# zhuwsh/ORB-SLAM2

Measured on AMD Instinct MI355X. Metric: frames/sec ORB extract+match, 1241x376 @1000 feats; bit-exact vs CPU, higher is better.
Workload: dtype u8; 1 GPU; KITTI-shape stereo 1241x376, nFeatures=1000/eye, 8 levels, FAST 20/7: extract(L)+extract(R)+ComputeStereoMatches; 1 frame = 1 stereo pair; images RESIDENT IN HBM when the timed region starts (kernel throughput: excludes PCIe; fed from pinned host memory the same path runs at config.host_fed_batched_frames_per_s -- the PCIe Gen5 x16 link, 0.96 MB per frame -- and one camera stream at config.host_fe; parallelism=1 independent camera-stream batches, one per GPU, ranks_seen=1, backend=none

## Files before the change

### include/orbx.h

```cpp
#ifndef ORBX_H
#define ORBX_H
#include <stddef.h>
#include <stdint.h>

#ifdef __cplusplus
extern "C" {
#endif

#define ORBX_OK 0
#define ORBX_E_INVALID (-1)
#define ORBX_E_CAPACITY (-2)
#define ORBX_E_TOO_SMALL (-3)
#define ORBX_E_NO_DEVICE (-4)
#define ORBX_E_HIP (-5)

typedef struct {
    float x, y, size, angle, response;
    int32_t octave, class_id;
} orbx_keypoint;

typedef struct orbx_extractor orbx_extractor;

const char *orbx_last_error(void);
int orbx_device_count(void);
// ... 231 lines not shown

int orbx_search_by_projection_keyframe(int device, const orbx_frame_feats *cur, const orbx_proj_points *pts,
                                       const float *scale_factors, int nlevels, float th, int orb_dist,
                                       int check_orientation, int32_t *match_cur, int *nmatches);
int orbx_search_by_projection_sim3(int device, const orbx_frame_feats *kf, const orbx_proj_points *pts,
                                   const float *scale_factors, int nlevels, float th, int32_t *match_kf, int *nmatches);
int orbx_window_best(int device, const orbx_frame_feats *kf, const orbx_proj_points *pts, const float *scale_factors,
                     const float *inv_sigma2, int nlevels, float th, int chi2, int max_dist, int32_t *best_idx,
                     int32_t *best_dist, int *nfound);
int orbx_search_by_sim3(int device, const orbx_frame_feats *kf1, const orbx_frame_feats *kf2, const orbx_proj_points *pts12,
                        const orbx_proj_points *pts21, const float *scale_factors1, const float *scale_factors2, int nlevels,
                        float th, int32_t *match12, int *nfound);

int orbx_search_for_initialization(int device, const orbx_frame_feats *f1, const orbx_frame_feats *f2,
                                   const float *prev_matched_xy, int window_size, float nnratio, int check_orientation,
                                   int32_t *matches12, int *nmatches);

int orbx_undistort_keypoints(int device, const float *xy, int n, float fx, float fy, float cx, float cy,
                             const float *dist_coef, int ndist, float *xy_out);


int orbx_distinctive_descriptors(int device, const uint8_t *desc, const int32_t *off, int npoints, int32_t *best_idx);


enum { ORBX_STAGE_RESIZE = 0, ORBX_STAGE_FAST = 1, ORBX_STAGE_TREE = 2, ORBX_STAGE_DESC = 3,
       ORBX_STAGE_STEREO = 4, ORBX_STAGE_STEREO_CUT = 5, ORBX_STAGE_COUNT = 6 };
int orbx_profile_enable(orbx_extractor *e, int enable);
int orbx_profile_stages(orbx_extractor *e, unsigned stage_mask);
int orbx_profile_read(orbx_extractor *e, float *ms, int *launches, int reset);

int orbx_debug_candidates(orbx_extractor *e, int image_index, int level, int32_t *x, int32_t *y, int32_t *resp, int cap, int *n);
int orbx_debug_level_counts(orbx_extractor *e, int image_index, int32_t *counts );
int orbx_debug_fast_form(const orbx_extractor *e);
int orbx_debug_set_bow_form(int form);
int orbx_debug_set_match_items(int in_memory);
int orbx_debug_match_timing(double *out4);

#ifdef __cplusplus
}
#endif
#endif
```

### orb-slam2_amd/csrc/orbx_extract.hip

```cpp
#include "orbx_device.h"
#include <atomic>
#include "orb_pattern.inc"

#include <math.h>
#include <stdio.h>
#include <stdlib.h>
#include <string.h>
#include <chrono>

__constant__ uint32_t c_pat4[256];
__constant__ uint4 c_omask[64];

#define RS_PX 4
#define RS_TW (64 * RS_PX)
#ifndef RS_TH_LOG2
#define RS_TH_LOG2 3
#endif
#define RS_TH (1 << RS_TH_LOG2)
#define RS_NT 64
#define RS_PITCH 320
#define RS_ROWS (RS_TH == 16 ? 22 : 12)

struct ResizeArgs {
    int d_w, d_pitch, s_w, s_pitch, s_level0;
// ... 49 lines not shown
    asm volatile("s_waitcnt vmcnt(0)" ::: "memory");
    __syncthreads();
    const int d_w = A.d_w, d_pitch = A.d_pitch;
    int hp[RS_PX], hc[RS_PX];
#pragma unroll
    for (int i = 0; i < RS_PX; i++) hp[i] = hc[i] = 0;
    uint8_t *dcol = dst + x4;
#define EMIT(Y, B0, B1, HA) do { \
        const unsigned w0_ = (unsigned)(B0) << 16, w1_ = (unsigned)(B1) << 16; \
        uint32_t out_ = 0; \
        _Pragma("unroll") for (int i = 0; i < RS_PX; i++) out_ |= ((__umulhi(w0_, (unsigned)(HA)[i]) + __umulhi(w1_, (unsigned)hc[i]) + 2u) >> 2) << (8 * i); \
        if (x4 < d_w) *reinterpret_cast<uint32_t *>(dcol + (long long)(Y) * d_pitch) = out_; } while (0)
#pragma unroll
    for (int k = 0; k < RS_ROWS; k++) {
        if (k < nrows) {
#pragma unroll
            for (int i = 0; i < RS_PX; i++) {
                hp[i] = hc[i];
                hc[i] = (src_t[k * RS_PITCH + o0[i]] * a0[i] + src_t[k * RS_PITCH + o1[i]] * a1[i]) >> 4;
            }
            const int e = __builtin_amdgcn_readfirstlane((int)qs[k].x);
            if (e >= 0) {
                const int y = e & 0xFFF;
                if (!(e & 0x1000)) {
                    const int b0 = __builtin_amdgcn_readfirstlane((int)qs[k].y), b1 = __builtin_amdgcn_readfirstlane((int)qs[k].z);
                    if (e & 0x2000) EMIT(y, b0, b1, hc);
                    else EMIT(y, b0, b1, hp);
                }
                if (e & 0x4000) EMIT(y + 1, 2048, 0, hc);
            }
        }
    }
#undef EMIT
}

__global__ __launch_bounds__(256) void k_resize_direct(const Geom *__restrict__ g, int l, PyrRef pr,
                                                       uint8_t *__restrict__ pyr_w, const int16_t *__restrict__ tabs)
{
    const LevelGeom &D = g->lv[l];
    const LevelGeom &S = g->lv[l - 1];
    const int b = blockIdx.z;
    const int x4 = (blockIdx.x * 64 + (threadIdx.x & 63)) * 4;
    const int y = blockIdx.y * 4 + (threadIdx.x >> 6);
    if (y >= D.h || x4 >= D.pitch) return;
    int spitch;
    const uint8_t *src = orbx_level_ptr(pr, S, l - 1, b, &spitch);
    uint8_t *dst = pyr_w + (long long)b * pr.pyr_stride + D.pyr_off;
    if (D.resize_lds == 2) {
        const uint8_t *r0 = src + (long long)(2 * y) * spitch, *r1 = r0 + spitch;
        uint32_t out = 0;
#pragma unroll
        for (int i = 0; i < 4; i++) {
            const int x = x4 + i;
            if (x < D.w) out |= (uint32_t)((r0[2 * x] + r0[2 * x + 1] + r1[2 * x] + r1[2 * x + 1] + 2) >> 2) << (8 * i);
        }
        *reinterpret_cast<uint32_t *>(dst + (long long)y * D.pitch + x4) = out;
        return;
    }
    const int16_t *tx = tabs + D.tab_x, *ty = tabs + D.tab_y;
    const int sy0 = ty[4 * y], b0 = ty[4 * y + 1], b1 = ty[4 * y + 2];
    const int sy1 = sy0 + 1 < S.h ? sy0 + 1 : S.h - 1;
    const uint8_t *r0 = src + (long long)sy0 * spitch, *r1 = src + (long long)sy1 * spitch;
    uint32_t out = 0;
#pragma unroll
    for (int i = 0; i < 4; i++) {
        const int x = x4 + i;
// ... 1765 lines not shown
            std::vector<int> ext(n + 1, 0);
            for (int t = 0; t < tiles; t++)
                for (int k = 0; k <= n; k++) {
                    const size_t i = (size_t)k * tiles + t;
                    int16_t *r = &tabs[off + ((size_t)t * (n + 1) + k) * rec];
                    if (hi[i] > 32767) return false;
                    r[0] = (int16_t)lo[i]; r[1] = (int16_t)hi[i]; r[2] = (int16_t)own[i];
                    int extent = hi[i] - lo[i];
                    if (!axis) {
                        int div;
                        if (k == 0) {
                            const int pitch_lim = lo[i] + (((dim(first - 1) - lo[i]) + 3) & ~3);
                            const int ndw = (std::min(lo[i] + ((hi[i] - lo[i] + 3) & ~3), pitch_lim) - lo[i]) / 4;
                            r[3] = (int16_t)ndw; div = ndw; extent = 4 * ndw;
                        } else { div = (extent + 3) >> 2; extent = (extent + 3) & ~3; }
                        const unsigned magic = (unsigned)((0x100000000ull + (unsigned)div - 1) / (unsigned)div);
                        r[4] = (int16_t)(magic & 0xFFFF); r[5] = (int16_t)(magic >> 16);
                    }
                    ext[k] = std::max(ext[k], extent);
                }
            if (!axis) P.tiles_x = tiles; else P.tiles_y = tiles;
            ext_axis[axis] = ext;
        }
        for (int k = 0; k < n; k++) lds[k & 1] = std::max(lds[k & 1], (size_t)ext_axis[0][k] * ext_axis[1][k]);
        P.lds_b = (int)align_up(lds[0], 16);
        P.lds_bytes = P.lds_b + (int)align_up(lds[1], 16);
        if (P.lds_bytes > PG_LDS_LIMIT) return false;
        first += n; gi++;
    }
    e->n_pyr_groups = gi;
    return true;
}

int orbx_prepare_geometry(orbx_extractor *e, int w, int h)
{
    if (e->geom.w == w && e->geom.h == h) return ORBX_OK;
    if (w > e->max_w || h > e->max_h || w > ORBX_MAX_DIM || h > ORBX_MAX_DIM) {
        orbx_set_error("image %dx%d exceeds the extractor's maximum %dx%d", w, h, e->max_w, e->max_h);
        return ORBX_E_INVALID;
    }
    Geom G;
    memset(&G, 0, sizeof G);
    G.nlevels = e->nlevels; G.w = w; G.h = h;
    size_t tab_units = 0;
    for (int l = 0; l < e->nlevels; l++) {
        LevelGeom &L = G.lv[l];
        L.w = orbx_cv_round((float)w * e->isf[l]);
        L.h = orbx_cv_round((float)h * e->isf[l]);
        const int min_b = ORBX_MIN_BORDER, max_bx = L.w - ORBX_EDGE + 3, max_by = L.h - ORBX_EDGE + 3;
        const float width = (float)(max_bx - min_b), height = (float)(max_by - min_b);
        if (max_bx - min_b < 30 || max_by - min_b < 30) {
            orbx_set_error("level %d (%dx%d) is smaller than one 30-px FAST cell", l, L.w, L.h);
            return ORBX_E_TOO_SMALL;
        }
        L.n_cols = (int)(width / 30.f);
        L.n_rows = (int)(height / 30.f);
        L.w_cell = (int)ceilf(width / L.n_cols);
        L.h_cell = (int)ceilf(height / L.n_rows);
        if (L.w_cell > 59 || L.h_cell > 59) { orbx_set_error("internal: cell larger than 59"); return ORBX_E_INVALID; }
        L.n_cells = L.n_cols * L.n_rows;
        L.cell_base = G.total_cells;
        G.total_cells += L.n_cells;
        L.cand_cap = ((L.w_cell + 1) / 2) * ((L.h_cell + 1) / 2);
        L.cand_off = G.cand_total;
        G.cand_total += (long long)L.n_cells * L.cand_cap;
        L.quota = e->quota[l];
// ... 78 lines not shown
        }
        for (int y0 = 0; y0 < L.h && ok; y0 += RS_TH) {
            const int yl = (y0 + RS_TH < L.h ? y0 + RS_TH : L.h) - 1;
            const int smax = ty[4 * yl] + 1 < S.h - 1 ? ty[4 * yl] + 1 : S.h - 1;
            if (smax - ty[4 * y0] + 1 > RS_ROWS) ok = false;
        }
        L.resize_lds = (S.w == 2 * L.w && S.h == 2 * L.h) ? 2 : (ok && emit_ok[l] && L.h < 4096) ? 1 : 0;
        if (L.resize_lds != 1) continue;
        for (int by = 0, y0 = 0; y0 < L.h; by++, y0 += RS_TH) {
            int16_t *r = &tabs[L.tab_ty + (size_t)by * RS_TY_REC];
            const int yl = (y0 + RS_TH < L.h ? y0 + RS_TH : L.h) - 1;
            const int sy_min = ty[4 * y0], sy_max = ty[4 * yl] + 1 < S.h - 1 ? ty[4 * yl] + 1 : S.h - 1, nrows = sy_max - sy_min + 1;
            r[0] = (int16_t)sy_min; r[1] = (int16_t)nrows; r[2] = r[3] = 0;
            for (int k = 0; k < RS_ROWS; k++) {
                int16_t *q = r + 4 + 4 * k;
                q[0] = -1; q[1] = q[2] = q[3] = 0;
                if (k >= nrows) continue;
                const int16_t *t = &emit[l][4 * (size_t)(sy_min + k)];
                if (t[0] < 0) continue;
                const int y = t[0] & 0xFFF, in1 = y >= y0 && y <= yl, in2 = (t[0] & 0x4000) && y + 1 >= y0 && y + 1 <= yl;
                if (!in1 && !in2) continue;
                q[0] = (int16_t)(y | (t[0] & 0x2000) | (in1 ? 0 : 0x1000) | (in2 ? 0x4000 : 0)); q[1] = t[1]; q[2] = t[2];
            }
        }
        for (int bx = 0, x0 = 0; x0 < L.w; bx++, x0 += RS_TW) {
            int16_t *r = &tabs[L.tab_tx + 4 * (size_t)bx];
            const int xl = (x0 + RS_TW < L.w ? x0 + RS_TW : L.w) - 1;
            const int sx_min = tx[4 * x0], sx_max = tx[4 * xl] + 1 < S.w - 1 ? tx[4 * xl] + 1 : S.w - 1, need = sx_max - sx_min + 1;
            const int nfull = std::min((need + 15) >> 4, (S.w - sx_min) >> 4), tail = std::max(need - 16 * nfull, 0);
            r[0] = (int16_t)sx_min; r[1] = (int16_t)nfull; r[2] = (int16_t)tail; r[3] = 0;
        }
    }
    if (!build_pyr_groups(e, G, tabs)) e->n_pyr_groups = 0;
    std::vector<CellRec> cells(G.total_cells);
    for (int l = 0; l < e->nlevels; l++) {
        const LevelGeom &L = G.lv[l];
        const int max_bx = L.w - ORBX_MIN_BORDER, max_by = L.h - ORBX_MIN_BORDER;
        for (int ci = 0; ci < L.n_cells; ci++) {
            CellRec &c = cells[L.cell_base + ci];
            const int row = ci / L.n_cols, col = ci % L.n_cols;
            const int ini_y = ORBX_MIN_BORDER + row * L.h_cell, ini_x = ORBX_MIN_BORDER + col * L.w_cell;
            const int max_y = ini_y + L.h_cell + 6 < max_by ? ini_y + L.h_cell + 6 : max_by;
            const int max_x = ini_x + L.w_cell + 6 < max_bx ? ini_x + L.w_cell + 6 : max_bx;
            c.level = (short)l;
            c.ini_x = (short)ini_x; c.ini_y = (short)ini_y; c.tw = (short)(max_x - ini_x); c.th = (short)(max_y - ini_y);
            c.skip = (ini_y >= max_by - 3 || ini_x >= max_bx - 6 || c.tw - 6 <= 0 || c.th - 6 <= 0) ? 1 : 0;
            c.pitch = L.pitch; c.cand_cap = L.cand_cap; c.pyr_off = L.pyr_off;
            { const int gpr = (c.tw - 6 + 3) >> 2; c.gpr_magic = gpr > 0 ? 0xFFFFFFFFu / (unsigned)gpr + 1u : 0u; }
            c.cand_slot = L.cand_off + (long long)ci * L.cand_cap;
        }
    }
    std::vector<PairRec> pairs;
    {
        bool ok = true;
        for (int l = 0; l < e->nlevels; l++) if (G.lv[l].w_cell > 32 || G.lv[l].h_cell > 56) ok = false;
        G.fast2_ok = ok ? 1 : 0;
        G.total_pairs = 0;
        if (ok) {
            for (int grp = 0; grp < 2; grp++) {
                int max_th = 0, max_dh = 0;
                G.fast2_first[grp] = (int)pairs.size();
                for (int l = 0; l < e->nlevels; l++) {
                    const LevelGeom &L = G.lv[l];
                    if ((L.h_cell <= 32 ? 0 : 1) != grp) continue;
                    max_th = std::max(max_th, L.h_cell + 6); max_dh = std::max(max_dh, L.h_cell);
                    for (int row = 0; row < L.n_rows; row++)
// ... 162 lines not shown
        max_w < 1 || max_h < 1 || ini_th < 1 || min_th < 1 || ini_th > 255 || min_th > ini_th) {
        orbx_set_error("orbx_extractor_create: invalid parameter");
        return ORBX_E_INVALID;
    }
    int ndev = 0;
    if (hipGetDeviceCount(&ndev) != hipSuccess || ndev < 1 || device < 0 || device >= ndev) {
        orbx_set_error("no usable HIP device (requested %d of %d); liborbx has no CPU fallback", device, ndev);
        return ORBX_E_NO_DEVICE;
    }
    ORBX_HIP(hipSetDevice(device));
    orbx_extractor *e = new orbx_extractor();
    e->prof_mask = ~0u;
    orbx_extractor_set_cv_profile(e, ORBX_CV_PROFILE_3_2);
    e->device = device; e->nfeatures = nfeatures; e->nlevels = nlevels; e->ini_th = ini_th; e->min_th = min_th;
    e->scale_factor = scale_factor; e->max_w = max_w; e->max_h = max_h; e->max_batch = max_batch;
    {
        const char *env = getenv("ORBX_PYR_GROUP_MAX_IMAGES");
        e->pyr_group_max_images = env && *env ? atoi(env) : 8;
        const char *mid = getenv("ORBX_PYR_GROUP_MID_IMAGES");
        e->pyr_group_mid_images = e->pyr_group_mid_cfg = mid && *mid ? atoi(mid) : 24;
        const char *kpw = getenv("ORBX_STEREO_KPW");
        e->stereo_kpw_forced = kpw && (*kpw == '1' || *kpw == '4') ? *kpw - '0' : 0;
        const char *pl = getenv("ORBX_PIPE_LANES"), *pi = getenv("ORBX_PIPE_INLINE");
        e->pipe_lanes = pl && *pl >= '1' && *pl <= '0' + ORBX_PIPE_DEPTH ? *pl - '0' : ORBX_PIPE_DEPTH;
        e->pipe_inline = !(pi && *pi == '0');
        const char *pk = getenv("ORBX_PIPE_KCOPY");
        e->pipe_kcopy = !(pk && *pk == '0');
        const char *pg = getenv("ORBX_PIPE_RGBD_GATHER");
        e->pipe_rgbd_gather = !(pg && *pg == '0');
        const char *fw = getenv("ORBX_FAST_WAVES");
        e->fast_waves = fw && *fw >= '1' && *fw <= '4' ? *fw - '0' : 0;
        const char *fp = getenv("ORBX_FAST_PAIR");
        e->fast_pair = fp && *fp == '1' ? 1 : 0;
    }
    e->sf[0] = 1.0f; e->sig2[0] = 1.0f;
    for (int i = 1; i < nlevels; i++) { e->sf[i] = (float)(e->sf[i - 1] * e->scale_factor); e->sig2[i] = e->sf[i] * e->sf[i]; }
    for (int i = 0; i < nlevels; i++) { e->isf[i] = 1.0f / e->sf[i]; e->isig2[i] = 1.0f / e->sig2[i]; }
    float factor = (float)(1.0f / e->scale_factor);
    float n_desired = nfeatures * (1 - factor) / (1 - (float)pow((double)factor, (double)nlevels));
    int sum = 0;
    for (int l = 0; l < nlevels - 1; l++) { e->quota[l] = orbx_cv_round(n_desired); sum += e->quota[l]; n_desired *= factor; }
    e->quota[nlevels - 1] = nfeatures - sum > 0 ? nfeatures - sum : 0;
    {
        int v, v0, vmax = (int)floor(15 * sqrtf(2.f) / 2 + 1), vmin = (int)ceil(15 * sqrtf(2.f) / 2);
        const double hp2 = 15 * 15;
        for (v = 0; v <= vmax; ++v) e->umax[v] = (int)lrint(sqrt(hp2 - v * v));
        for (v = 15, v0 = 0; v >= vmin; --v) { while (e->umax[v0] == e->umax[v0 + 1]) ++v0; e->umax[v] = v0; ++v0; }
    }
    hipError_t he = hipStreamCreateWithFlags(&e->stream, hipStreamNonBlocking);
    if (he != hipSuccess) { orbx_set_error("hipStreamCreate failed: %s", hipGetErrorString(he)); delete e; return ORBX_E_HIP; }
    int rc = upload_constants(e);
    if (rc == ORBX_OK && hipMalloc((void **)&e->d_geom, sizeof(Geom)) != hipSuccess) { orbx_set_error("hipMalloc failed"); rc = ORBX_E_HIP; }
    if (rc == ORBX_OK && hipMalloc((void **)&e->d_lvl_cnt, sizeof(int) * (size_t)max_batch * ORBX_MAX_LEVELS + 16) != hipSuccess) { orbx_set_error("hipMalloc failed"); rc = ORBX_E_HIP; }
    if (rc == ORBX_OK && hipHostMalloc((void **)&e->h_flag, 64, hipHostMallocDefault) != hipSuccess) { orbx_set_error("hipHostMalloc failed"); rc = ORBX_E_HIP; }
    if (rc != ORBX_OK) { orbx_extractor_destroy(e); return rc; }
    *e->h_flag = 0;
    hipMemset(e->d_lvl_cnt, 0, sizeof(int) * (size_t)max_batch * ORBX_MAX_LEVELS + 16);
    *out = e;
    return ORBX_OK;
}

extern "C" void orbx_debug_pipe_prof_print();
extern "C" void orbx_extractor_destroy(orbx_extractor *e)
{
    if (!e) return;
    hipSetDevice(e->device);
// ... 101 lines not shown
    const int regime = e->n_pyr_groups > 0 && batch <= e->pyr_group_max_images ? 2
                     : e->n_pyr_groups > 1 && batch <= e->pyr_group_mid_images ? 1 : 0;
    auto launch_level = [&](int l) {
        const LevelGeom &L = G.lv[l];
        orbx_prof_begin(e, ORBX_STAGE_RESIZE, s);
        if (L.resize_lds == 1)
        {
            const LevelGeom &S = G.lv[l - 1];
            ResizeArgs ra;
            ra.d_w = L.w; ra.d_pitch = L.pitch; ra.s_w = S.w; ra.s_pitch = S.pitch; ra.s_level0 = l == 1;
            ra.tab_x = L.tab_x; ra.tab_tx = L.tab_tx; ra.tab_ty = L.tab_ty; ra.d_off = L.pyr_off; ra.s_off = S.pyr_off;
            hipLaunchKernelGGL(k_resize, dim3(batch, (L.w + RS_TW - 1) / RS_TW, (L.h + RS_TH - 1) / RS_TH), dim3(RS_NT), 0, s, ra, pr, e->d_pyr, e->d_tabs);
        }
        else
            hipLaunchKernelGGL(k_resize_direct, dim3((L.pitch / 4 + 63) / 64, (L.h + 3) / 4, batch), dim3(256), 0, s,
                               e->d_geom, l, pr, e->d_pyr, e->d_tabs);
        orbx_prof_end(e, s);
    };
    auto launch_group = [&](int gi) {
        const orbx_extractor::PyrGroup &P = e->pyr_groups[gi];
        const LevelGeom &S = G.lv[P.first - 1];
        PyrGroupArgs ga;
        memset(&ga, 0, sizeof ga);
        ga.n = P.n; ga.s_level0 = P.first == 1; ga.s_w = S.w; ga.s_h = S.h; ga.s_pitch = S.pitch; ga.s_off = S.pyr_off;
        ga.tab_cx = P.tab_cx; ga.tab_cy = P.tab_cy; ga.lds_b = P.lds_b;
        for (int k = 0; k < P.n; k++) {
            const LevelGeom &L = G.lv[P.first + k];
            ga.lv[k].w = L.w; ga.lv[k].h = L.h; ga.lv[k].pitch = L.pitch; ga.lv[k].tab_x = L.tab_x; ga.lv[k].tab_y = L.tab_y; ga.lv[k].pyr_off = L.pyr_off;
        }
        orbx_prof_begin(e, ORBX_STAGE_RESIZE, s);
        hipLaunchKernelGGL(k_pyr_group, dim3(P.tiles_x, P.tiles_y, batch), dim3(PG_NT), (size_t)P.lds_bytes, s, ga, pr, e->d_pyr, e->d_tabs);
        orbx_prof_end(e, s);
    };
    if (regime == 0) for (int l = 1; l < G.nlevels; l++) launch_level(l);
    else
        for (int gi = 0; gi < e->n_pyr_groups; gi++) {
            if (regime == 2 || gi >= 1) launch_group(gi);
            else for (int l = e->pyr_groups[gi].first; l < e->pyr_groups[gi].first + e->pyr_groups[gi].n; l++) launch_level(l);
        }
    orbx_prof_begin(e, ORBX_STAGE_FAST, s);
    e->last_fast_form = 1;
    {
        FastArgs fa;
        fa.total_cells = G.total_cells; fa.lds_sc = G.fast_lds_sc; fa.lds_list = G.fast_lds_list; fa.lds_bm = G.fast_lds_bm;
        fa.bm_rows = G.fast_bm_rows; fa.ini_th = e->ini_th; fa.min_th = e->min_th; fa.cand_total = G.cand_total; fa.list_cap = ORBX_FAST_LIST_CAP;
        const dim3 grid((G.total_cells + 8 * FAST_XG - 1) / (8 * FAST_XG) * (8 * FAST_XG), batch);
        if (G.fast_small)
        {
            const long long waves1 = (long long)G.total_cells * batch;
            const int nw = e->fast_waves ? e->fast_waves : waves1 * 4 <= 16384 ? 4 : waves1 * 2 <= 16384 ? 2 : 1;
            int lds_bytes = G.fast_lds_bytes;
            if (nw > 1) { fa.list_cap = G.fast_list_cap_big; fa.lds_bm = G.fast_lds_bm_big; lds_bytes = G.fast_lds_bytes_big; }
            if (G.fast2_ok && e->fast_pair == 1) {
                e->last_fast_form = 2;
                fa.list_cap = FAST2_LIST_CAP;
                for (int grp = 0; grp < 2; grp++) {
                    if (!G.fast2_count[grp]) continue;
                    fa.lds_sc = G.fast2_lds_sc[grp]; fa.lds_list = G.fast2_lds_list[grp]; fa.lds_bm = G.fast2_lds_bm[grp]; fa.bm_rows = G.fast2_bm_rows[grp];
                    const dim3 grid2((G.fast2_count[grp] + 8 * FAST_XG - 1) / (8 * FAST_XG) * (8 * FAST_XG), batch);
                    hipLaunchKernelGGL((k_fast2<FAST2_P, FAST2_SP>), grid2, dim3(64), G.fast2_lds_bytes[grp], s, fa, (const PairRec *)e->d_pairs + G.fast2_first[grp],
                                       G.fast2_count[grp], pr, e->d_cell_cnt, e->d_cand, e->d_cand_prim);
                }
            } else
#define LAUNCH_FAST(NW_) hipLaunchKernelGGL((k_fast<48, 40, NW_>), grid, dim3(64 * NW_), lds_bytes, s, fa, e->d_cells, pr, e->d_cell_cnt, e->d_cand, e->d_cand_prim)
            if (nw == 4) LAUNCH_FAST(4); else if (nw == 3) LAUNCH_FAST(3); else if (nw == 2) LAUNCH_FAST(2);
            else if (grid.x <= 65535) hipLaunchKernelGGL((k_fast<48, 40, 1, true>), dim3(batch, grid.x), dim3(64), lds_bytes, s, fa, e->d_cells, pr, e->d_cell_cnt, e->d_cand, e->d_cand_prim);
            else LAUNCH_FAST(1);
#undef LAUNCH_FAST
        }
        else
            hipLaunchKernelGGL((k_fast<ORBX_TILE_PITCH, ORBX_SCORE_PITCH, 1>), grid, dim3(64), G.fast_lds_bytes, s, fa, e->d_cells, pr, e->d_cell_cnt,
// ... 740 lines not shown
    if (!e || !kps || !desc || !n_out || ticket < 0) { orbx_set_error("orbx_extract_wait: invalid argument"); return ORBX_E_INVALID; }
    return pipe_wait(e, ticket, 1, kps, desc, cap, n_out, nullptr, nullptr);
}

extern "C" int orbx_extract(orbx_extractor *e, const uint8_t *img, int w, int h, size_t stride,
                            orbx_keypoint *kps, uint8_t *desc, int cap, int *n_out)
{
    const uint8_t *imgs[1] = { img };
    if (!img && w > 0 && h > 0) { orbx_set_error("img is NULL"); return ORBX_E_INVALID; }
    return orbx_extract_batch(e, imgs, 1, w, h, stride, kps, desc, cap, n_out);
}

extern "C" int orbx_pyramid_level(orbx_extractor *e, int image_index, int level, uint8_t *dst, size_t dst_stride, int *w, int *h)
{
    if (!e || !e->geom.w || !e->last_img0 || level < 0 || level >= e->nlevels || image_index < 0 || image_index >= e->last_batch) {
        orbx_set_error("orbx_pyramid_level: no pyramid / bad index");
        return ORBX_E_INVALID;
    }
    const LevelGeom &L = e->geom.lv[level];
    if (w) *w = L.w;
    if (h) *h = L.h;
    if (!dst) return ORBX_OK;
    if (dst_stride < (size_t)L.w) { orbx_set_error("dst_stride < level width"); return ORBX_E_INVALID; }
    ORBX_HIP(orbx_use_device(e->device));
    ORBX_HIP(hipStreamSynchronize(e->stream));
    const uint8_t *src; size_t pitch;
    if (level == 0) { src = e->last_img0 + e->last_img_stride * image_index; pitch = e->last_pitch; }
    else { src = e->d_pyr + (size_t)e->geom.pyr_bytes * image_index + L.pyr_off; pitch = L.pitch; }
    ORBX_HIP(hipMemcpy2D(dst, dst_stride, src, pitch, L.w, L.h, hipMemcpyDeviceToHost));
    return ORBX_OK;
}

extern "C" int orbx_debug_fast_form(const orbx_extractor *e) { return e ? e->last_fast_form : ORBX_E_INVALID; }

extern "C" int orbx_debug_level_counts(orbx_extractor *e, int image_index, int32_t *counts)
{
    if (!e || !counts || image_index < 0 || image_index >= e->last_batch) { orbx_set_error("bad argument"); return ORBX_E_INVALID; }
    ORBX_HIP(orbx_use_device(e->device));
    ORBX_HIP(hipStreamSynchronize(e->stream));
    ORBX_HIP(hipMemcpy(counts, e->d_lvl_cnt + (size_t)image_index * ORBX_MAX_LEVELS, sizeof(int) * e->nlevels, hipMemcpyDeviceToHost));
    return ORBX_OK;
}

extern "C" int orbx_debug_candidates(orbx_extractor *e, int image_index, int level, int32_t *x, int32_t *y, int32_t *resp, int cap, int *n)
{
    if (!e || !n || !e->geom.w || level < 0 || level >= e->nlevels || image_index < 0 || image_index >= e->last_batch) {
        orbx_set_error("bad argument");
        return ORBX_E_INVALID;
    }
    ORBX_HIP(orbx_use_device(e->device));
    ORBX_HIP(hipStreamSynchronize(e->stream));
    const Geom &G = e->geom;
    const LevelGeom &L = G.lv[level];
    std::vector<int> cnt(L.n_cells);
    std::vector<uint32_t> slots((size_t)L.n_cells * L.cand_cap);
    ORBX_HIP(hipMemcpy(cnt.data(), e->d_cell_cnt + (size_t)image_index * G.total_cells + L.cell_base, sizeof(int) * L.n_cells, hipMemcpyDeviceToHost));
    ORBX_HIP(hipMemcpy(slots.data(), e->d_cand + (size_t)image_index * G.cand_total + L.cand_off, slots.size() * 4, hipMemcpyDeviceToHost));
    std::vector<uint32_t> prim((size_t)L.n_cells * ORBX_CAND_PRIM);
    ORBX_HIP(hipMemcpy(prim.data(), e->d_cand_prim + ((size_t)image_index * G.total_cells + L.cell_base) * ORBX_CAND_PRIM, prim.size() * 4, hipMemcpyDeviceToHost));
    int k = 0;
    for (int c = 0; c < L.n_cells; c++)
        for (int i = 0; i < cnt[c]; i++, k++)
            if (k < cap && x && y && resp) {
                const uint32_t p = i < ORBX_CAND_PRIM ? prim[(size_t)c * ORBX_CAND_PRIM + i] : slots[(size_t)c * L.cand_cap + i];
                x[k] = p & 0xFFF; y[k] = (p >> 12) & 0xFFF; resp[k] = p >> 24;
            }
// ... 16 lines not shown
```

### orb-slam2_amd/csrc/orbx_internal.h

```cpp
#pragma once
#include <hip/hip_runtime.h>
#include <stdint.h>
#include <string>
#include <vector>
#include "../../include/orbx.h"

#define ORBX_MAX_LEVELS 16
#define ORBX_EDGE 19
#define ORBX_MIN_BORDER 16
#define ORBX_TILE_PITCH 80
#define ORBX_SCORE_PITCH 64
#define ORBX_MAX_DIM 4096
#define ORBX_NODE_BITS 14
#define ORBX_CAND_PRIM 16
#ifndef ORBX_TREE_REG_PTS
#define ORBX_TREE_REG_PTS 3072
#endif
#define ORBX_TREE_REG_PTS_BIG 4096
#ifndef ORBX_TREE_OVER_PTS
#define ORBX_TREE_OVER_PTS 1024
#endif
#define ORBX_FAST_LIST_CAP 512

struct LevelGeom {
// ... 77 lines not shown
    CellRec *d_cells; size_t cells_cap;
    void *d_pairs; size_t pairs_cap;
    int last_fast_form;
    int fast_pair;
    uint8_t *d_pyr; size_t pyr_cap;
    uint8_t *d_stage_in; size_t stage_in_cap;
    int *d_cell_cnt; size_t cell_cnt_cap;
    uint32_t *d_cand; size_t cand_cap;
    uint32_t *d_cand_prim; size_t cand_prim_cap;
    uint32_t *d_tree_pts; uint16_t *d_tree_nid; size_t tree_cap;
    unsigned char *d_tree_tab; size_t tree_tab_cap;
    int *d_lvl_cnt;
    uint32_t *d_lvl_kp; size_t lvl_kp_cap;
    uint8_t *h_stage_in; size_t h_stage_in_cap;
    uint8_t *h_out; size_t h_out_cap;
    int *h_flag;
    void *d_out_kps, *d_out_desc, *d_out_n; int out_cap; int out_batch;
    float *d_out_ur, *d_out_depth;
    int *d_st_dist; size_t st_cap;
    void *d_st_entries; size_t st_ent_cap;
    void *scratch[10]; size_t scratch_cap[10];
    PipeSlot pipe[ORBX_PIPE_DEPTH]; hipStream_t copy_in, copy_out; unsigned pipe_next;
    int pipe_warm_w, pipe_warm_h;
    int pipe_rgbd_warm_w, pipe_rgbd_warm_h;
    bool pipe_rgbd_gather;
    bool pipe_counted;
    orbx_extractor *lanes[ORBX_PIPE_DEPTH - 1];
    int pipe_lanes;
    bool pipe_inline;
    bool pipe_kcopy;
    int *flag_out;
    struct PyrGroup { int first, n, tiles_x, tiles_y, tab_cx, tab_cy, lds_b, lds_bytes; } pyr_groups[ORBX_MAX_LEVELS];
    int n_pyr_groups;
    int pyr_group_max_images;
    int pyr_group_mid_images;
    int pyr_group_mid_cfg;
    int stereo_kpw_forced;
    int fast_waves;
    int *d_rt_off; size_t rt_off_cap; uint8_t *d_rt_entries; size_t rt_entries_cap; int rt_ent_cap;
    const void *rt_kps; int rt_cap, rt_batch;
    int *d_st_arrive;
    const uint8_t *last_img0; size_t last_img_stride, last_pitch; int last_batch;
    bool prof, prof_chain; unsigned prof_mask; hipStream_t prof_last_stream; std::vector<ProfEvent> prof_ev; std::vector<hipEvent_t> prof_pool;
    float prof_ms[ORBX_STAGE_COUNT]; int prof_n[ORBX_STAGE_COUNT];
};

struct DevFeat {
    int n, nnodes;
    const uint32_t *desc;
    const uint32_t *node_id;
    const int32_t *node_off;
    const uint32_t *feat;
    const uint8_t *flag;
    const float *angle, *x, *y, *u_right;
    const int32_t *octave;
    const uint32_t *sdesc;
    const uint8_t *sflag;
};

struct orbx_bow_frames {
    int device, batch, cap, npad;
    uint8_t *d_buf;
    uint32_t *word_id; double *word_w; uint32_t *node_id;
    uint32_t *bow_id; double *bow_val; int *counts;
    uint32_t *fv_node_id; int32_t *fv_node_off; uint32_t *fv_feat;
    float *angle;
// ... 43 lines not shown
```

### orb-slam2_amd/orbx.py

```python
import ctypes as C
import os
import numpy as np

_HERE = os.path.dirname(os.path.abspath(__file__))
_SO = os.environ.get("ORBX_SO") or os.path.join(_HERE, "liborbx.so")

KP_DTYPE = np.dtype([("x", "<f4"), ("y", "<f4"), ("size", "<f4"), ("angle", "<f4"),
                     ("response", "<f4"), ("octave", "<i4"), ("class_id", "<i4")])
STAGES = ("resize", "fast", "tree", "desc", "stereo", "stereo_cut")


class OrbxError(RuntimeError):
    def __init__(self, code, msg):
        super().__init__(f"orbx error {code}: {msg}")
        self.code = code


class FeatSet(C.Structure):
    _fields_ = [("n", C.c_int), ("desc", C.c_void_p), ("nnodes", C.c_int), ("node_id", C.c_void_p),
                ("node_off", C.c_void_p), ("feat", C.c_void_p), ("flag", C.c_void_p), ("angle", C.c_void_p),
                ("x", C.c_void_p), ("y", C.c_void_p), ("octave", C.c_void_p), ("u_right", C.c_void_p)]


class FrameFeats(C.Structure):
# ... 156 lines not shown
    L.orbx_frame_size.argtypes = [vp]
    L.orbx_frame_read.argtypes = [vp, vp, vp, vp, vp, vp, vp]
    L.orbx_frame_destroy.argtypes = [vp]; L.orbx_frame_destroy.restype = None
    L.orbx_frame_search_by_projection_last_frame.argtypes = [vp, vp, C.POINTER(ProjPoints), vp, i, f, i, f, i, vp, ip]
    L.orbx_frame_search_by_projection_map_points.argtypes = [vp, vp, C.POINTER(ProjPoints), vp, i, f, f, vp, ip]
    L.orbx_frame_search_by_projection_keyframe.argtypes = [vp, vp, C.POINTER(ProjPoints), vp, i, f, i, i, vp, ip]
    L.orbx_bow_frames_create.argtypes = [i, i, i, C.POINTER(vp)]
    L.orbx_bow_frames_destroy.argtypes = [vp]; L.orbx_bow_frames_destroy.restype = None
    L.orbx_bow_transform_batch_device.argtypes = [vp, vp, vp, vp, vp, i, i, vp]
    L.orbx_bow_frames_read.argtypes = [vp, i, vp, vp, vp, ip, vp, vp, vp, ip]
    L.orbx_bowdb_search_batch_device.argtypes = [vp, vp, i, f, i, vp, vp, vp]
    L.orbx_bowdb_search_batch_device_compact.argtypes = [vp, vp, i, f, i, vp, i, vp, vp]
    L.orbx_undistort_keypoints.argtypes = [i, vp, i, f, f, f, f, vp, i, vp]
    L.orbx_rectifier_create.argtypes = [i, i, i, i, i, vp, vp, C.POINTER(vp)]
    L.orbx_rectifier_destroy.argtypes = [vp]; L.orbx_rectifier_destroy.restype = None
    L.orbx_rectifier_size.argtypes = [vp, ip, ip]
    L.orbx_remap_batch_device.argtypes = [vp, vp, C.c_size_t, C.c_size_t, i, vp, C.c_size_t, C.c_size_t, vp]
    L.orbx_extract_rectified.argtypes = [vp, vp, vp, i, i, C.c_size_t, vp, vp, i, ip, vp, C.c_size_t]
    RP = C.POINTER(RGBDParamsStruct)
    L.orbx_extract_rgbd.argtypes = [vp, vp, i, i, sz, i, i, vp, sz, RP, vp, vp, i, ip, vp, vp, vp]
    L.orbx_extract_rgbd_submit.argtypes = [vp, vp, i, i, sz, i, i, vp, sz, RP, ip]
    L.orbx_extract_rgbd_wait.argtypes = [vp, i, vp, vp, i, ip, vp, vp, vp]
    L.orbx_rgbd_depth_batch_device.argtypes = [i, vp, vp, i, i, vp, sz, sz, i, i, RP, vp, vp, vp, vp]
    L.orbx_search_for_initialization.argtypes = [i, C.POINTER(FrameFeats), C.POINTER(FrameFeats), vp, i, f, i, vp, ip]
    L.orbx_search_by_sim3.argtypes = [i, C.POINTER(FrameFeats), C.POINTER(FrameFeats), C.POINTER(ProjPoints), C.POINTER(ProjPoints),
                                      vp, vp, i, f, vp, ip]
    L.orbx_distinctive_descriptors.argtypes = [i, vp, vp, i, vp]
    L.orbx_profile_enable.argtypes = [vp, i]
    L.orbx_profile_stages.argtypes = [vp, C.c_uint]
    L.orbx_profile_read.argtypes = [vp, vp, vp, i]
    L.orbx_debug_candidates.argtypes = [vp, i, i, vp, vp, vp, i, ip]
    L.orbx_debug_level_counts.argtypes = [vp, i, vp]
    L.orbx_debug_fast_form.argtypes = [vp]
    L.orbx_debug_set_bow_form.argtypes = [i]
    L.orbx_debug_set_match_items.argtypes = [i]
    L.orbx_debug_match_timing.argtypes = [vp]
    _lib = L
    return L


def device_identity(device):
    buf = C.create_string_buffer(160)
    _check(lib().orbx_device_identity(int(device), buf, len(buf)))
    return buf.value.decode(errors="replace")


def pipeline_depth():
    return lib().orbx_pipeline_depth()


class _Pinned:
    def __init__(self, nbytes):
        self.ptr = lib().orbx_pinned_alloc(nbytes)
        if not self.ptr:
            raise OrbxError(-5, lib().orbx_last_error().decode(errors="replace"))

    def __del__(self):
        if getattr(self, "ptr", None):
            lib().orbx_pinned_free(self.ptr); self.ptr = None


def pinned_array(shape, dtype=np.uint8):
    nbytes = int(np.prod(shape)) * np.dtype(dtype).itemsize
    owner = _Pinned(nbytes)
    buf = (C.c_uint8 * nbytes).from_address(owner.ptr)
    buf._orbx_owner = owner
# ... 45 lines not shown
    s.flag = arr("flag", np.uint8); s.angle = arr("angle", np.float32)
    s.x = arr("x", np.float32); s.y = arr("y", np.float32)
    s.octave = arr("octave", np.int32); s.u_right = arr("u_right", np.float32)
    return s, keep


class ORBextractor:

    def __init__(self, nfeatures, scaleFactor, nlevels, iniThFAST, minThFAST, device=0, max_size=(4096, 4096), max_batch=1):
        self._L = lib()
        self._h = C.c_void_p()
        self.nfeatures, self.nlevels, self.max_batch, self.device = nfeatures, nlevels, max_batch, device
        self._pipe_shapes, self._pipe_last = {}, (max_size[0], max_size[1])
        _check(self._L.orbx_extractor_create(C.byref(self._h), nfeatures, scaleFactor, nlevels, iniThFAST, minThFAST,
                                             device, max_size[0], max_size[1], max_batch))

    def __del__(self):
        h = getattr(self, "_h", None)
        if h:
            self._L.orbx_extractor_destroy(h)
            self._h = None

    def set_cv_profile(self, profile):
        _check(self._L.orbx_extractor_set_cv_profile(self._h, profile))

    def set_pyramid_group_limit(self, max_images):
        _check(self._L.orbx_extractor_set_pyramid_group_limit(self._h, int(max_images)))

    def pipeline_warm(self, w, h):
        _check(self._L.orbx_pipeline_warm(self._h, int(w), int(h)))

    def debug_fast_form(self):
        return self._L.orbx_debug_fast_form(self._h)

    def GetLevels(self): return self._L.orbx_get_levels(self._h)
    def GetScaleFactor(self): return self._L.orbx_get_scale_factor(self._h)

    def _tables(self):
        t = [np.zeros(self.nlevels, np.float32) for _ in range(4)]
        _check(self._L.orbx_get_scale_tables(self._h, *[_p(a) for a in t]))
        return t

    def GetScaleFactors(self): return self._tables()[0]
    def GetInverseScaleFactors(self): return self._tables()[1]
    def GetScaleSigmaSquares(self): return self._tables()[2]
    def GetInverseScaleSigmaSquares(self): return self._tables()[3]

    def GetFeaturesPerLevel(self):
        q = np.zeros(self.nlevels, np.int32)
        _check(self._L.orbx_get_features_per_level(self._h, _p(q)))
        return q

    def max_keypoints(self, w, h):
        n = self._L.orbx_max_keypoints(self._h, w, h)
        if n < 0:
            _check(n)
        return n

    def __call__(self, image, mask=None):
        image = np.asarray(image)
        if image.size == 0:
            return np.zeros(0, KP_DTYPE), np.zeros((0, 32), np.uint8)
        if image.dtype != np.uint8 or image.ndim != 2:
            raise OrbxError(-1, "image must be 2-D uint8 (CV_8UC1, reference src/ORBextractor.cc:1269)")
        if image.strides[1] != 1:
            image = np.ascontiguousarray(image)
# ... 620 lines not shown
```

Measured before the change: 159,200 frames/s.

## Fuse consecutive pyramid resize levels into a single two-level kernel

```diff
diff --git a/include/orbx.h b/include/orbx.h
--- a/include/orbx.h
+++ b/include/orbx.h
@@ -287,6 +287,7 @@
 int orbx_debug_candidates(orbx_extractor *e, int image_index, int level, int32_t *x, int32_t *y, int32_t *resp, int cap, int *n);
 int orbx_debug_level_counts(orbx_extractor *e, int image_index, int32_t *counts );
 int orbx_debug_fast_form(const orbx_extractor *e);
+int orbx_debug_pyramid_pairs(const orbx_extractor *e);
 int orbx_debug_set_bow_form(int form);
 int orbx_debug_set_match_items(int in_memory);
 int orbx_debug_match_timing(double *out4);
diff --git a/orb-slam2_amd/csrc/orbx_extract.hip b/orb-slam2_amd/csrc/orbx_extract.hip
--- a/orb-slam2_amd/csrc/orbx_extract.hip
+++ b/orb-slam2_amd/csrc/orbx_extract.hip
@@ -105,6 +105,149 @@
         }
     }
 #undef EMIT
+}
+
+#define R2_OW 208
+#ifndef R2_TH
+#define R2_TH 10
+#endif
+#define R2_IROWS ((R2_TH * 6 + 4) / 5 + 2)
+#define R2_SROWS ((R2_IROWS * 6 + 4) / 5 + 2)
+#define R2_IPITCH 256
+#ifndef ORBX_PYR_PAIR_PLAN_DEFAULT
+#define ORBX_PYR_PAIR_PLAN_DEFAULT ((1 << 1) | (1 << 3) | (1 << 5))
+#endif
+#define R2_CX_REC 8
+#define R2_RY_REC (8 + 4 * (R2_SROWS + R2_IROWS))
+static_assert(R2_IROWS * R2_IPITCH <= R2_SROWS * RS_PITCH, "level-l rows share the source buffer");
+struct Resize2Args {
+    int w1, pitch1, w2, pitch2, s_w, s_pitch, s_level0;
+    int tab_x1, tab_x2, tab_cx, tab_ry;
+    long long off1, off2, s_off;
+};
+
+__global__ __launch_bounds__(RS_NT) void k_resize2(const Resize2Args A, PyrRef pr,
+                                                 uint8_t *__restrict__ pyr_w, const int16_t *__restrict__ tabs)
+{
+    __shared__ __align__(16) uint8_t src_t[R2_SROWS * RS_PITCH];
+    const int b = blockIdx.x, lane = threadIdx.x, tile_x = blockIdx.y, tile_y = blockIdx.z;
+    const int spitch = A.s_level0 ? pr.img0_pitch : A.s_pitch;
+    const uint8_t *src = A.s_level0 ? pr.img0 + (long long)b * pr.img0_stride : pr.pyr + (long long)b * pr.pyr_stride + A.s_off;
+    uint8_t *dst1 = pyr_w + (long long)b * pr.pyr_stride + A.off1, *dst2 = pyr_w + (long long)b * pr.pyr_stride + A.off2;
+    const int16_t *ry = tabs + A.tab_ry + tile_y * R2_RY_REC, *rx = tabs + A.tab_cx + R2_CX_REC * tile_x;
+    const int sy_min = __builtin_amdgcn_readfirstlane((int)ry[0]), nrows = __builtin_amdgcn_readfirstlane((int)ry[1]);
+    const int ly = __builtin_amdgcn_readfirstlane((int)ry[2]), own_y = __builtin_amdgcn_readfirstlane((int)ry[3]);
+    const int sx_min = __builtin_amdgcn_readfirstlane((int)rx[0]), nfull = __builtin_amdgcn_readfirstlane((int)rx[1]),
+              tail = __builtin_amdgcn_readfirstlane((int)rx[2]), lo = __builtin_amdgcn_readfirstlane((int)rx[3]),
+              hi = __builtin_amdgcn_readfirstlane((int)rx[4]), own_x = __builtin_amdgcn_readfirstlane((int)rx[5]),
+              xl2 = __builtin_amdgcn_readfirstlane((int)rx[6]);
+    short4 qs[R2_SROWS];
+#pragma unroll
+    for (int k = 0; k < R2_SROWS; k++) qs[k] = *reinterpret_cast<const short4 *>(ry + 8 + 4 * k);
+    const int x1 = lo + RS_PX * lane;
+    short4 qx[RS_PX];
+#pragma unroll
+    for (int i = 0; i < RS_PX; i++) qx[i] = *reinterpret_cast<const short4 *>(tabs + A.tab_x1 + 4 * min(x1 + i, hi - 1));
+    {
+        const uint8_t *s0 = src + (long long)sy_min * spitch + sx_min;
+        const int lr = lane / 20, lc = lane - lr * 20;
+        if (lr < 3 && lc < nfull)
+            for (int r = 0; r < nrows; r += 3)
+                if (r + lr < nrows)
+                    __builtin_amdgcn_global_load_lds(reinterpret_cast<const uint32_t *>(s0 + (long long)(r + lr) * spitch + 16 * lc),
+                                                     reinterpret_cast<uint32_t *>(src_t + r * RS_PITCH), 16, 0, 0);
+        if (tail)
+            for (int i = lane; i < nrows * tail; i += RS_NT) {
+                const int r = i / tail, c = 16 * nfull + (i - r * tail);
+                src_t[r * RS_PITCH + c] = s0[(long long)r * spitch + c];
+            }
+    }
+    int o0[RS_PX], o1[RS_PX], a0[RS_PX], a1[RS_PX];
+#pragma unroll
+    for (int i = 0; i < RS_PX; i++) {
+        const int sx0 = qx[i].x;
+        o0[i] = sx0 - sx_min;
+        o1[i] = min(sx0 + 1, A.s_w - 1) - sx_min;
+        a0[i] = qx[i].y;
+        a1[i] = qx[i].z;
+    }
+    asm volatile("s_waitcnt vmcnt(0)" ::: "memory");
+    __syncthreads();
+    int hp[RS_PX], hc[RS_PX];
+#pragma unroll
+    for (int i = 0; i < RS_PX; i++) hp[i] = hc[i] = 0;
+    const bool own_c = x1 < own_x;
+    uint8_t *dcol1 = dst1 + x1;
+#define EMIT1(Y, B0, B1, HA) do { \
+        const unsigned w0_ = (unsigned)(B0) << 16, w1_ = (unsigned)(B1) << 16; \
+        uint32_t out_ = 0; \
+        _Pragma("unroll") for (int i = 0; i < RS_PX; i++) out_ |= ((__umulhi(w0_, (unsigned)(HA)[i]) + __umulhi(w1_, (unsigned)hc[i]) + 2u) >> 2) << (8 * i); \
+        *reinterpret_cast<uint32_t *>(src_t + ((Y) - ly) * R2_IPITCH + RS_PX * lane) = out_; \
+        if ((Y) < own_y && own_c) *reinterpret_cast<uint32_t *>(dcol1 + (long long)(Y) * A.pitch1) = out_; } while (0)
+#pragma unroll
+    for (int k = 0; k < R2_SROWS; k++) {
+        if (k < nrows) {
+#pragma unroll
+            for (int i = 0; i < RS_PX; i++) {
+                hp[i] = hc[i];
+                hc[i] = (src_t[k * RS_PITCH + o0[i]] * a0[i] + src_t[k * RS_PITCH + o1[i]] * a1[i]) >> 4;
+            }
+            const int e = __builtin_amdgcn_readfirstlane((int)qs[k].x);
+            if (e >= 0) {
+                const int y = e & 0xFFF;
+                if (!(e & 0x1000)) {
+                    const int b0 = __builtin_amdgcn_readfirstlane((int)qs[k].y), b1 = __builtin_amdgcn_readfirstlane((int)qs[k].z);
+                    if (e & 0x2000) EMIT1(y, b0, b1, hc);
+                    else EMIT1(y, b0, b1, hp);
+                }
+                if (e & 0x4000) EMIT1(y + 1, 2048, 0, hc);
+            }
+        }
+    }
+#undef EMIT1
+    short4 qt[R2_IROWS];
+#pragma unroll
+    for (int k = 0; k < R2_IROWS; k++) qt[k] = *reinterpret_cast<const short4 *>(ry + 8 + 4 * R2_SROWS + 4 * k);
+    const int x2 = tile_x * R2_OW + RS_PX * lane;
+#pragma unroll
+    for (int i = 0; i < RS_PX; i++) qx[i] = *reinterpret_cast<const short4 *>(tabs + A.tab_x2 + 4 * min(x2 + i, xl2));
+#pragma unroll
+    for (int i = 0; i < RS_PX; i++) {
+        const int sx0 = qx[i].x;
+        o0[i] = sx0 - lo;
+        o1[i] = min(sx0 + 1, A.w1 - 1) - lo;
+        a0[i] = qx[i].y;
+        a1[i] = qx[i].z;
+        hp[i] = hc[i] = 0;
+    }
+    __syncthreads();
+    const bool st2 = lane < R2_OW / RS_PX && x2 < A.w2;
+    uint8_t *dcol2 = dst2 + x2;
+#define EMIT2(Y, B0, B1, HA) do { \
+        const unsigned w0_ = (unsigned)(B0) << 16, w1_ = (unsigned)(B1) << 16; \
+        uint32_t out_ = 0; \
+        _Pragma("unroll") for (int i = 0; i < RS_PX; i++) out_ |= ((__umulhi(w0_, (unsigned)(HA)[i]) + __umulhi(w1_, (unsigned)hc[i]) + 2u) >> 2) << (8 * i); \
+        if (st2) *reinterpret_cast<uint32_t *>(dcol2 + (long long)(Y) * A.pitch2) = out_; } while (0)
+#pragma unroll
+    for (int k = 0; k < R2_IROWS; k++) {
+        const int e = __builtin_amdgcn_readfirstlane((int)qt[k].x);
+        if (e == -2) break;
+#pragma unroll
+        for (int i = 0; i < RS_PX; i++) {
+            hp[i] = hc[i];
+            hc[i] = (src_t[k * R2_IPITCH + o0[i]] * a0[i] + src_t[k * R2_IPITCH + o1[i]] * a1[i]) >> 4;
+        }
+        if (e >= 0) {
+            const int y = e & 0xFFF;
+            if (!(e & 0x1000)) {
+                const int b0 = __builtin_amdgcn_readfirstlane((int)qt[k].y), b1 = __builtin_amdgcn_readfirstlane((int)qt[k].z);
+                if (e & 0x2000) EMIT2(y, b0, b1, hc);
+                else EMIT2(y, b0, b1, hp);
+            }
+            if (e & 0x4000) EMIT2(y + 1, 2048, 0, hc);
+        }
+    }
+#undef EMIT2
 }
 
 __global__ __launch_bounds__(256) void k_resize_direct(const Geom *__restrict__ g, int l, PyrRef pr,
@@ -1936,6 +2079,79 @@
     return true;
 }
 
+static void build_pyr_pair(orbx_extractor *e, const Geom &G, int l, const std::vector<std::vector<int16_t>> &emit, std::vector<int16_t> &tabs)
+{
+    orbx_extractor::PyrPair &P = e->pyr_pair[l];
+    P.ok = 0;
+    if (l + 1 >= G.nlevels) return;
+    const LevelGeom &S = G.lv[l - 1], &I = G.lv[l], &O = G.lv[l + 1];
+    if (I.resize_lds != 1 || O.resize_lds != 1) return;
+    const int16_t *txI = &tabs[I.tab_x], *tyI = &tabs[I.tab_y], *txO = &tabs[O.tab_x], *tyO = &tabs[O.tab_y];
+    const int tiles_x = (O.w + R2_OW - 1) / R2_OW, tiles_y = (O.h + R2_TH - 1) / R2_TH;
+    std::vector<int16_t> cx((size_t)tiles_x * R2_CX_REC, 0), ry((size_t)tiles_y * R2_RY_REC, 0);
+    std::vector<int> lo(tiles_x), nhi(tiles_x);
+    for (int t = 0; t < tiles_x; t++) {
+        const int xl = std::min((t + 1) * R2_OW, O.w) - 1;
+        lo[t] = txO[4 * (t * R2_OW)] & ~3;
+        nhi[t] = std::min(txO[4 * xl] + 1, I.w - 1) + 1;
+        if (t ? lo[t] < lo[t - 1] : lo[t] != 0) return;
+    }
+    for (int t = 0; t < tiles_x; t++) {
+        const int own = t + 1 < tiles_x ? lo[t + 1] : I.w, hi = std::max(nhi[t], own);
+        if (hi - lo[t] > R2_IPITCH) return;
+        const int sx_min = txI[4 * lo[t]], sx_max = std::min(txI[4 * (hi - 1)] + 1, S.w - 1), need = sx_max - sx_min + 1;
+        const int nfull = std::min((need + 15) >> 4, (S.w - sx_min) >> 4), tail = std::max(need - 16 * nfull, 0);
+        if (need > RS_PITCH || sx_min < 0) return;
+        int16_t *r = &cx[(size_t)t * R2_CX_REC];
+        r[0] = (int16_t)sx_min; r[1] = (int16_t)nfull; r[2] = (int16_t)tail; r[3] = (int16_t)lo[t]; r[4] = (int16_t)hi; r[5] = (int16_t)own;
+        r[6] = (int16_t)(std::min((t + 1) * R2_OW, O.w) - 1);
+    }
+    std::vector<int> ly(tiles_y), nhy(tiles_y);
+    for (int t = 0; t < tiles_y; t++) {
+        const int yl = std::min((t + 1) * R2_TH, O.h) - 1;
+        ly[t] = tyO[4 * (t * R2_TH)];
+        nhy[t] = std::min(tyO[4 * yl] + 1, I.h - 1) + 1;
+        if (t ? ly[t] < ly[t - 1] : ly[t] != 0) return;
+    }
+    for (int t = 0; t < tiles_y; t++) {
+        const int own_y = t + 1 < tiles_y ? ly[t + 1] : I.h, hy = std::max(nhy[t], own_y), y0 = ly[t], y1 = hy - 1;
+        if (hy - y0 > R2_IROWS) return;
+        const int sy_min = tyI[4 * y0], sy_max = std::min(tyI[4 * y1] + 1, S.h - 1), nrows = sy_max - sy_min + 1;
+        if (nrows > R2_SROWS || sy_min < 0) return;
+        int16_t *r = &ry[(size_t)t * R2_RY_REC];
+        r[0] = (int16_t)sy_min; r[1] = (int16_t)nrows; r[2] = (int16_t)y0; r[3] = (int16_t)own_y;
+        for (int k = 0; k < R2_SROWS; k++) {
+            int16_t *q = r + 8 + 4 * k;
+            q[0] = -1;
+            if (k >= nrows) continue;
+            const int16_t *te = &emit[l][4 * (size_t)(sy_min + k)];
+            if (te[0] < 0) continue;
+            const int y = te[0] & 0xFFF, in1 = y >= y0 && y <= y1, in2 = (te[0] & 0x4000) && y + 1 >= y0 && y + 1 <= y1;
+            if (!in1 && !in2) continue;
+            if ((in2 ? y + 1 : y) - y0 > k && k != nrows - 1) return;
+            q[0] = (int16_t)(y | (te[0] & 0x2000) | (in1 ? 0 : 0x1000) | (in2 ? 0x4000 : 0)); q[1] = te[1]; q[2] = te[2];
+        }
+        const int Y0 = t * R2_TH, Yl = std::min(Y0 + R2_TH, O.h) - 1;
+        int last = -1;
+        for (int k = 0; k < R2_IROWS; k++) {
+            int16_t *q = r + 8 + 4 * R2_SROWS + 4 * k;
+            q[0] = -1;
+            if (k >= hy - y0) continue;
+            const int16_t *te = &emit[l + 1][4 * (size_t)(y0 + k)];
+            if (te[0] < 0) continue;
+            const int y = te[0] & 0xFFF, in1 = y >= Y0 && y <= Yl, in2 = (te[0] & 0x4000) && y + 1 >= Y0 && y + 1 <= Yl;
+            if (!in1 && !in2) continue;
+            q[0] = (int16_t)(y | (te[0] & 0x2000) | (in1 ? 0 : 0x1000) | (in2 ? 0x4000 : 0)); q[1] = te[1]; q[2] = te[2];
+            last = k;
+        }
+        for (int k = last + 1; k < R2_IROWS; k++) r[8 + 4 * R2_SROWS + 4 * k] = -2;
+    }
+    tabs.resize(align_up(tabs.size(), 4));
+    P.tab_cx = (int)tabs.size(); tabs.insert(tabs.end(), cx.begin(), cx.end());
+    P.tab_ry = (int)tabs.size(); tabs.insert(tabs.end(), ry.begin(), ry.end());
+    P.tiles_x = tiles_x; P.tiles_y = tiles_y; P.ok = 1;
+}
+
 int orbx_prepare_geometry(orbx_extractor *e, int w, int h)
 {
     if (e->geom.w == w && e->geom.h == h) return ORBX_OK;
@@ -2080,6 +2296,7 @@
         }
     }
     if (!build_pyr_groups(e, G, tabs)) e->n_pyr_groups = 0;
+    for (int l = 1; l < e->nlevels; l++) build_pyr_pair(e, G, l, emit, tabs);
     std::vector<CellRec> cells(G.total_cells);
     for (int l = 0; l < e->nlevels; l++) {
         const LevelGeom &L = G.lv[l];
@@ -2308,6 +2525,19 @@
         e->fast_waves = fw && *fw >= '1' && *fw <= '4' ? *fw - '0' : 0;
         const char *fp = getenv("ORBX_FAST_PAIR");
         e->fast_pair = fp && *fp == '1' ? 1 : 0;
+        const char *pp = getenv("ORBX_PYR_PAIRS");
+        e->pyr_pairs = pp && (*pp == '0' || *pp == '1') ? *pp - '0' : -1;
+        const char *plan = getenv("ORBX_PYR_PAIR_PLAN");
+        e->pyr_pair_plan = ORBX_PYR_PAIR_PLAN_DEFAULT;
+        if (plan && *plan) {
+            e->pyr_pair_plan = 0;
+            for (const char *q = plan; *q; ) {
+                const int l = atoi(q);
+                if (l >= 1 && l < ORBX_MAX_LEVELS) e->pyr_pair_plan |= 1 << l;
+                while (*q && *q != ',') q++;
+                if (*q == ',') q++;
+            }
+        }
     }
     e->sf[0] = 1.0f; e->sig2[0] = 1.0f;
     for (int i = 1; i < nlevels; i++) { e->sf[i] = (float)(e->sf[i - 1] * e->scale_factor); e->sig2[i] = e->sf[i] * e->sf[i]; }
@@ -2475,11 +2705,29 @@
         hipLaunchKernelGGL(k_pyr_group, dim3(P.tiles_x, P.tiles_y, batch), dim3(PG_NT), (size_t)P.lds_bytes, s, ga, pr, e->d_pyr, e->d_tabs);
         orbx_prof_end(e, s);
     };
-    if (regime == 0) for (int l = 1; l < G.nlevels; l++) launch_level(l);
+    e->last_pyr_pairs = 0;
+    const bool pairs = e->pyr_pairs == 1 || (e->pyr_pairs < 0 && e->pyr_group_max_images > 0);
+    auto launch_levels = [&](int first, int end) {
+        for (int l = first; l < end; ) {
+            const orbx_extractor::PyrPair &P = e->pyr_pair[l];
+            if (!pairs || !(e->pyr_pair_plan >> l & 1) || !P.ok || l + 1 >= end) { launch_level(l++); continue; }
+            const LevelGeom &S = G.lv[l - 1], &I = G.lv[l], &O = G.lv[l + 1];
+            Resize2Args ra;
+            ra.w1 = I.w; ra.pitch1 = I.pitch; ra.w2 = O.w; ra.pitch2 = O.pitch; ra.s_w = S.w; ra.s_pitch = S.pitch; ra.s_level0 = l == 1;
+            ra.tab_x1 = I.tab_x; ra.tab_x2 = O.tab_x; ra.tab_cx = P.tab_cx; ra.tab_ry = P.tab_ry;
+            ra.off1 = I.pyr_off; ra.off2 = O.pyr_off; ra.s_off = S.pyr_off;
+            orbx_prof_begin(e, ORBX_STAGE_RESIZE, s);
+            hipLaunchKernelGGL(k_resize2, dim3(batch, P.tiles_x, P.tiles_y), dim3(RS_NT), 0, s, ra, pr, e->d_pyr, e->d_tabs);
+            orbx_prof_end(e, s);
+            e->last_pyr_pairs |= 1 << l;
+            l += 2;
+        }
+    };
+    if (regime == 0) launch_levels(1, G.nlevels);
     else
         for (int gi = 0; gi < e->n_pyr_groups; gi++) {
             if (regime == 2 || gi >= 1) launch_group(gi);
-            else for (int l = e->pyr_groups[gi].first; l < e->pyr_groups[gi].first + e->pyr_groups[gi].n; l++) launch_level(l);
+            else launch_levels(e->pyr_groups[gi].first, e->pyr_groups[gi].first + e->pyr_groups[gi].n);
         }
     orbx_prof_begin(e, ORBX_STAGE_FAST, s);
     e->last_fast_form = 1;
@@ -3286,6 +3534,7 @@
 }
 
 extern "C" int orbx_debug_fast_form(const orbx_extractor *e) { return e ? e->last_fast_form : ORBX_E_INVALID; }
+extern "C" int orbx_debug_pyramid_pairs(const orbx_extractor *e) { return e ? e->last_pyr_pairs : ORBX_E_INVALID; }
 
 extern "C" int orbx_debug_level_counts(orbx_extractor *e, int image_index, int32_t *counts)
 {
diff --git a/orb-slam2_amd/csrc/orbx_internal.h b/orb-slam2_amd/csrc/orbx_internal.h
--- a/orb-slam2_amd/csrc/orbx_internal.h
+++ b/orb-slam2_amd/csrc/orbx_internal.h
@@ -133,6 +133,10 @@
     int *flag_out;
     struct PyrGroup { int first, n, tiles_x, tiles_y, tab_cx, tab_cy, lds_b, lds_bytes; } pyr_groups[ORBX_MAX_LEVELS];
     int n_pyr_groups;
+    struct PyrPair { int ok, tiles_x, tiles_y, tab_cx, tab_ry; } pyr_pair[ORBX_MAX_LEVELS];
+    int pyr_pair_plan;
+    int last_pyr_pairs;
+    int pyr_pairs;
     int pyr_group_max_images;
     int pyr_group_mid_images;
     int pyr_group_mid_cfg;
diff --git a/orb-slam2_amd/orbx.py b/orb-slam2_amd/orbx.py
--- a/orb-slam2_amd/orbx.py
+++ b/orb-slam2_amd/orbx.py
@@ -212,6 +212,7 @@
     L.orbx_debug_candidates.argtypes = [vp, i, i, vp, vp, vp, i, ip]
     L.orbx_debug_level_counts.argtypes = [vp, i, vp]
     L.orbx_debug_fast_form.argtypes = [vp]
+    L.orbx_debug_pyramid_pairs.argtypes = [vp]
     L.orbx_debug_set_bow_form.argtypes = [i]
     L.orbx_debug_set_match_items.argtypes = [i]
     L.orbx_debug_match_timing.argtypes = [vp]
@@ -323,6 +324,10 @@
 
     def debug_fast_form(self):
         return self._L.orbx_debug_fast_form(self._h)
+
+    def debug_pyramid_pairs(self):
+        m = self._L.orbx_debug_pyramid_pairs(self._h)
+        return [l for l in range(1, 32) if m >> l & 1]
 
     def GetLevels(self): return self._L.orbx_get_levels(self._h)
     def GetScaleFactor(self): return self._L.orbx_get_scale_factor(self._h)
```

Result: faster. 161,100 frames/s, median of 6 (+1.2%).
